# quzefan/LuSh-NeRF

Hardware: AMD Instinct MI355X
Metric: training rays/sec (fwd+bwd), N_samples=64+64 (higher is better)
Workload: dtype f16 MFMA forward (one fp16 plane per operand, fp32 accumulate; render outputs within 3e-5 of the fp32 reference); backward fp16 MFMA (one plane, per-launch power-of-two loss scale), fp32 accumulate; 1 GPU; poster_lushnerf 1xMI355X N_rand=4096/GPU N_samples=64 N_importance=64 blur kernel (DSK/RBK) on, fwd+bwd+Adam, one RCCL all-reduce of the flat gradient (BASELINE config C2); rays_per_gpu=4096, marched_rays_per_gpu=20480, planes_fwd=fp16x1, parallelism=dp1

## Files before the change

lush_nerf_amd/csrc/lush_mlp_wide.hip:

```cpp
#include "lush_mlp_wide.h"
#include "lush_host.h"

#include <cstdio>
#include <cstdlib>
#include <utility>

namespace lush {

constexpr int WD_PE_PITCH = PE_ROW * 2 + 16;
constexpr int WD_PE_PLANE = WD_MT * WD_PE_PITCH;
constexpr int WD_SB = 2;
enum { WB_NONE = 0, WB_REG = 1, WB_PEX = 2, WB_PED = 3 };
enum { WC_NONE = 0, WC_ACT = 1, WC_ALPHA = 2 };

constexpr int WD_WRAP = NetNerf::fwd4_len / 8;
static_assert(NetNerf::fwd4_len % 8 == 0, "the quarter-row stream is whole positions");

LUSH_CLOCK_DECL(lush_clock_wide_fwd)

struct WdRt {
    bool pre_on;
    unsigned clamp;
    char* mptr[2];
    unsigned lane2;
    const float* nextbias;
    char* tile;
    char* srows;
    unsigned soff[2];
    unsigned srow_off;
};

typedef __attribute__((ext_vector_type(2))) unsigned short u16x2;
struct WdConvTmp {
    unsigned o[4];
    unsigned m;
    unsigned word[4];
};

template <int NRQP, int KB0, bool MASK>
struct WdConv {
    static constexpr int NB = 2 * NRQP;
    static constexpr int UPT = MASK ? 8 : 4;
    static constexpr int UPB = 2 * UPT;
    static constexpr int NVU = NB * UPB;

    template <int K>
    static __device__ __forceinline__ void unit(f32x16 (&pend)[2][2], u32x4 (&xout)[2][16], WdConvTmp& t, unsigned clamp) {
        constexpr int b = K / UPB, r = K % UPB, tt = r / UPT, u = r % UPT;
        constexpr int c = b % 2, rbl = b / 2, kb = KB0 + 2 * rbl + tt;
        constexpr int kind = MASK ? ((u == 0 || u == 1 || u == 3 || u == 5) ? 0 : 1) : 0;
        constexpr int i = MASK ? (kind == 0 ? (u == 0 ? 0 : (u == 1 ? 1 : (u == 3 ? 2 : 3))) : (u == 2 ? 0 : (u == 4 ? 1 : (u == 6 ? 2 : 3)))) : u;
        if constexpr (kind == 0) {
            unsigned o;
            asm volatile("v_cvt_pk_f16_f32 %0, %1, %2\n\tv_pk_max_i16 %0, %0, %3"
                         : "=&v"(o) : "v"(pend[c][rbl][8 * tt + 2 * i]), "v"(pend[c][rbl][8 * tt + 2 * i + 1]), "s"(clamp));
            t.o[i] = o;
            if constexpr (i == 3) {
                const u32x4 v = {t.o[0], t.o[1], t.o[2], t.o[3]};
                xout[c][kb] = v;
            }
        } else {
            constexpr int sh = 8 * tt + 2 * i;
            unsigned z;
            if constexpr (tt == 0 && i == 0) {
                asm volatile("v_pk_sub_u16 %0, 1, %1 op_sel_hi:[0,1] clamp" : "=v"(t.m) : "v"(t.o[i]));
            } else if constexpr (tt == 1 && i == 3) {
                unsigned w;
                asm volatile("v_pk_sub_u16 %1, 1, %3 op_sel_hi:[0,1] clamp\n\tv_lshl_or_b32 %2, %1, %4, %2\n\tv_lshrrev_b32 %1, 15, %2\n\tv_or_b32 %1, %1, %2\n\tv_not_b32 %0, %1"
                             : "=v"(w), "=&v"(z), "+v"(t.m) : "v"(t.o[i]), "n"(sh));
                t.word[b] = w;
            } else {
                asm volatile("v_pk_sub_u16 %0, 1, %2 op_sel_hi:[0,1] clamp\n\tv_lshl_or_b32 %1, %0, %3, %1" : "=&v"(z), "+v"(t.m) : "v"(t.o[i]), "n"(sh));
            }
        }
    }
};


template <int NRQ, int NPOS, int BMAIN, int KB0, int PRE, int CK, int NRQP, int CKB0, bool MASK, int NRQN, int D, int PQ, bool STASH, int LD>
struct WdPass {
    static constexpr int KBPP = 8 / NRQ;
    static constexpr int NG = NPOS * 16;
    static constexpr int DG = D < NG ? D : NG;
    using CV = WdConv<NRQP, CKB0, MASK>;
    static constexpr int NBLK = CK == WC_ACT ? CV::NB : 0;
    static constexpr int IPB = CK == WC_ACT ? CV::UPB + 5 : 0;
    static constexpr int NIT = NBLK * IPB;
    static_assert(BMAIN == WB_REG || NPOS == 1, "a PE-image segment is one position");
    static_assert(!STASH || NPOS == 4, "the stash pipeline is laid out over the 16 positions of a layer");

    struct Regs {
        bf16x8 a1[4];
        u32x4 bpe[2][4];
        WdConvTmp ct;
        unsigned dma_dst, dma_off;
    };

    static constexpr int ST_JOBS = 8;
    static constexpr bool st_write(int g) { return STASH && g % 16 >= 12 && (4 * PQ + g / 16) < ST_JOBS; }
    static constexpr bool st_read(int g) { return STASH && g % 16 >= 12 && (4 * PQ + g / 16) >= 1 && (4 * PQ + g / 16) <= ST_JOBS; }
    static constexpr int st_store_job(int g) {
        const int P = 4 * PQ + g / 16, m = g % 16;
        const int J = m >= 14 ? P - 1 : (m < 2 ? P - 2 : -1);
        return (STASH && J >= 0 && J < ST_JOBS) ? J : -1;
    }
    static constexpr int st_store_row(int g) { return g % 16 >= 14 ? g % 16 - 14 : g % 16 + 2; }
    static constexpr bool st_store(int g) { return st_store_job(g) >= 0; }

    static constexpr int item_weight(int k) {
        const int r = k % (IPB > 0 ? IPB : 1), b = k / (IPB > 0 ? IPB : 1);
        if (r < CV::UPB) {
            if (!MASK) return 3;
            const int u = r % CV::UPT;
            return (u == 0 || u == 1 || u == 3 || u == 5) ? 3 : 2;
        }
        if (r == CV::UPB) return MASK ? 2 : 0;
        return (b / 2) < NRQN ? 1 : 0;
    }
    static constexpr int fixed_load(int g) {
        const int m = g % 16;
        int w = 0;
        if (m < 4) w += 1;
        if (m == 4 || m == 5) w += 3;
        if (m == 8) w += 10;
        if (m >= 9 && m <= 11) w += 1;
        if (st_write(g)) w += 1;
        if (st_read(g)) w += 1;
        if (st_store(g)) w += 2;
        return w;
    }
    struct Sched {
        int first[NG + 1];
        int cap;
    };
    static constexpr Sched make_sched() {
        Sched S{};
        for (int cap = 6; cap < 64; ++cap) {
            int k = 0;
            for (int g = 0; g < NG; ++g) {
                S.first[g] = k;
                int load = fixed_load(g);
                if (g < DG || g == NG - 1) {
                    while (k < NIT) {
                        const int w = item_weight(k);
                        if (w > 0 && load + w > cap && !(g == NG - 1)) break;
                        load += w;
                        ++k;
                    }
                }
            }
            S.first[NG] = k;
            S.cap = cap;
            int last = 0;
            for (int g = 0; g < NG; ++g)
                if (S.first[g + 1] > S.first[g]) last = g;
            if (k == NIT && (last < DG || NIT == 0)) return S;
        }
        return S;
    }
    static constexpr Sched SC = make_sched();

    template <int SRC, int NKB>
    static __device__ __forceinline__ void load_bpe(Regs& r, const char* peimg, int row0, int lane) {
        const int n = lane & 31, hh = lane >> 5;
        const char* p = peimg + (row0 + n) * WD_PE_PITCH + hh * 16;
#pragma unroll
        for (int c = 0; c < 2; ++c)
#pragma unroll
            for (int k = 0; k < NKB; ++k)
                r.bpe[c][k] = *reinterpret_cast<const u32x4*>(p + c * 32 * WD_PE_PITCH + ((SRC == WB_PED ? PE_X / 8 : 0) + 2 * k) * 16);
    }

    template <int SRC, int NRQ_, int I, int M>
    static __device__ __forceinline__ void mfma(f32x16 (&act)[2][2], const Regs& r, const WdCarry& cr, const u32x4 (&xin)[2][16]) {
        constexpr int u = M / 2, c = M % 2;
        constexpr int kbl = NRQ_ == 2 ? u / 2 : u, rbl = NRQ_ == 2 ? u % 2 : 0;
        const bf16x8 a = u < 4 ? cr.a0[u] : r.a1[u - 4];
        if constexpr (SRC == WB_REG) act[c][rbl] = mfma_f16(a, __builtin_bit_cast(bf16x8, xin[c][KB0 + I * (8 / NRQ_) + kbl]), act[c][rbl]);
        else act[c][rbl] = mfma_f16(a, __builtin_bit_cast(bf16x8, r.bpe[c][SRC == WB_PED ? kbl % 2 : kbl]), act[c][rbl]);
    }

    template <int M>
    static __device__ __forceinline__ void fixed(WdCtx& cx, Regs& r, WdCarry& cr, const char* rd, const char* rd_next) {
        if constexpr (M < 4) {
            r.a1[M] = *reinterpret_cast<const bf16x8*>(rd + (4 + M) * 1024 + cx.lane * 16);
        } else if constexpr (M == 4) {
            r.dma_dst = cx.dma_base + cx.slot_off;
            r.dma_off = cx.fetch_off;
        } else if constexpr (M == 5) {
            cx.fetch_off = cx.fetch_off + WD_SLOT == (unsigned)WD_WRAP * WD_SLOT ? 0u : cx.fetch_off + WD_SLOT;
            cx.slot_off = cx.slot_off + WD_SLOT == (unsigned)WD_S * WD_SLOT ? 0u : cx.slot_off + WD_SLOT;
        } else if constexpr (M == 8) {
            wd_dma_pair(cx.gbase + r.dma_off, cx.gbase + r.dma_off + 4096u, cx.voff, r.dma_dst, r.dma_dst + 4096u);
            cr.a0[0] = *reinterpret_cast<const bf16x8*>(rd_next + cx.lane * 16);
        } else if constexpr (M >= 9 && M <= 11) {
            cr.a0[M - 8] = *reinterpret_cast<const bf16x8*>(rd_next + (M - 8) * 1024 + cx.lane * 16);
        }
    }

    template <int K>
    static __device__ __forceinline__ void item(f32x16 (&pend)[2][2], u32x4 (&xout)[2][16], Regs& r, const WdRt& rt, int lane) {
        constexpr int b = K / IPB, rr = K % IPB, c = b % 2, rbl = b / 2;
        if constexpr (rr < CV::UPB) {
            CV::template unit<b * CV::UPB + rr>(pend, xout, r.ct, rt.clamp);
        } else if constexpr (rr == CV::UPB) {
            if constexpr (MASK) *reinterpret_cast<unsigned short*>(rt.mptr[c] + rbl * 128 + rt.lane2) = (unsigned short)r.ct.word[b];
        } else if constexpr (rbl < NRQN) {
            constexpr int j = rr - CV::UPB;
            const f32x4 v = *reinterpret_cast<const f32x4*>(rt.nextbias + rbl * 32 + 8 * (lane >> 5) + (j == 1 ? 0 : j == 2 ? 4 : j == 3 ? 16 : 20));
#pragma unroll
            for (int e = 0; e < 4; ++e) pend[c][rbl][4 * (j - 1) + e] = v[e];
        }
    }

    template <int G>
    static __device__ __forceinline__ void pending(f32x16 (&pend)[2][2], u32x4 (&xout)[2][16], Regs& r, const WdRt& rt, int lane, float (&alpha)[2]) {
        if constexpr (CK == WC_ACT) {
            wd_unroll<SC.first[G], SC.first[G + 1]>([&](auto kc) __attribute__((always_inline)) { item<decltype(kc)::value>(pend, xout, r, rt, lane); });
        } else if constexpr (CK == WC_ALPHA) {
            if constexpr (G == 0) {
                alpha[0] = pend[0][0][0];
                alpha[1] = pend[1][0][0];
            }
            if constexpr (G == 1) {
                asm volatile("" ::"v"(pend[0][0]), "v"(pend[1][0]));
            }
            if constexpr (G >= 1 && G <= 8) {
                constexpr int q = G - 1, c = q % 2, rbl = (q / 2) % 2, jj = q / 4;
                if constexpr (rbl < NRQN) {
#pragma unroll
                    for (int j2 = 0; j2 < 2; ++j2) {
                        const int j = 1 + 2 * jj + j2;
                        const f32x4 v = *reinterpret_cast<const f32x4*>(rt.nextbias + rbl * 32 + 8 * (lane >> 5) + (j == 1 ? 0 : j == 2 ? 4 : j == 3 ? 16 : 20));
#pragma unroll
                        for (int e = 0; e < 4; ++e) pend[c][rbl][4 * (j - 1) + e] = v[e];
                    }
                }
            }
        }
    }

    template <int JOB, int I4>
    static __device__ __forceinline__ void stash_store(const WdCarry& cr, const WdRt& rt) {
        constexpr int c = JOB / 4, j = JOB % 4;
        __builtin_nontemporal_store(cr.sb[I4 % WD_SB], reinterpret_cast<u32x4*>(rt.srows + ((c * 32 + 8 * I4) * LD + j * 64) * 2 + rt.srow_off));
    }
    template <int G>
    static __device__ __forceinline__ void stash(const u32x4 (&xin)[2][16], WdCarry& cr, const WdRt& rt, int lane) {
        constexpr int P = 4 * PQ + G / 16, m = G % 16;
        if constexpr (st_store(G)) stash_store<st_store_job(G), st_store_row(G)>(cr, rt);
        if constexpr (st_write(G)) {
            constexpr int job = P, c = job / 4, j = job % 4, o = m - 12;
            const int n = lane & 31, hh = lane >> 5;
            *reinterpret_cast<u32x4*>(rt.tile + (job % 2) * 4096 + n * 128 + (((2 * o + hh) ^ (n & 7)) << 4)) = xin[c][4 * j + o];
        }
        if constexpr (st_read(G)) {
            constexpr int job = P - 1, i = m - 12;
            const int row = 8 * i + (lane >> 3);
            cr.sb[i % WD_SB] = *reinterpret_cast<const u32x4*>(rt.tile + (job % 2) * 4096 + row * 128 + (((lane & 7) ^ (row & 7)) << 4));
        }
    }

    static constexpr int stores_in(int g0, int g1) {
        int n = 0;
        for (int g = g0 < 0 ? 0 : g0; g < g1 && g < NG; ++g) {
            if (st_store(g)) ++n;
            if (CK == WC_ACT && MASK)
                for (int k = SC.first[g]; k < SC.first[g + 1]; ++k)
                    if (k % IPB == CV::UPB) ++n;
        }
        return n;
    }

    template <int SRC, int NRQ_, int I, bool MAIN>
    static __device__ __forceinline__ void position(WdCtx& cx, f32x16 (&act)[2][2], f32x16 (&pend)[2][2], const u32x4 (&xin)[2][16],
                                                    u32x4 (&xout)[2][16], Regs& r, WdCarry& cr, const char* peimg, int row0, const WdRt& rt,
                                                    float (&alpha)[2]) {
        if constexpr (SRC != WB_REG) load_bpe<SRC, (SRC == WB_PED ? 2 : 4)>(r, peimg, row0, cx.lane);
        const char* rd = cx.ring + cx.slot_off;
        __builtin_amdgcn_sched_barrier(0);
        wd_unroll<0, 8>([&](auto mc) __attribute__((always_inline)) {
            constexpr int M = decltype(mc)::value;
            mfma<SRC, NRQ_, I, M>(act, r, cr, xin);
            fixed<M>(cx, r, cr, rd, nullptr);
            if constexpr (MAIN) {
                stash<16 * I + M>(xin, cr, rt, cx.lane);
                pending<16 * I + M>(pend, xout, r, rt, cx.lane, alpha);
            }
            __builtin_amdgcn_sched_barrier(0);
        });
        constexpr int younger = 2 * (WD_S - 2) + (MAIN ? stores_in(16 * (I + 1 - WD_S) + 8, 16 * I + 8) : 0);
        wd_wait_vm<(younger < 63 ? younger : 63)>();
        lds_barrier();
        const char* rd_next = cx.ring + cx.slot_off;
        __builtin_amdgcn_sched_barrier(0);
        wd_unroll<8, 16>([&](auto mc) __attribute__((always_inline)) {
            constexpr int M = decltype(mc)::value;
            mfma<SRC, NRQ_, I, M>(act, r, cr, xin);
            fixed<M>(cx, r, cr, rd, rd_next);
            if constexpr (MAIN) {
                stash<16 * I + M>(xin, cr, rt, cx.lane);
                pending<16 * I + M>(pend, xout, r, rt, cx.lane, alpha);
            }
            __builtin_amdgcn_sched_barrier(0);
        });
    }

    static __device__ __forceinline__ void run(WdCtx& cx, f32x16 (&act)[2][2], f32x16 (&pend)[2][2], const u32x4 (&xin)[2][16],
                                               u32x4 (&xout)[2][16], WdCarry& cr, const char* peimg, int row0, const WdRt& rt, float (&alpha)[2]) {
        Regs r;
        if constexpr (PRE == WB_PEX) {
            if (rt.pre_on) position<WB_PEX, 2, 0, false>(cx, act, pend, xin, xout, r, cr, peimg, row0, rt, alpha);
        } else if constexpr (PRE == WB_PED) {
            position<WB_PED, 2, 0, false>(cx, act, pend, xin, xout, r, cr, peimg, row0, rt, alpha);
        }
        wd_unroll<0, NPOS>([&](auto ic) __attribute__((always_inline)) {
            position<BMAIN, NRQ, decltype(ic)::value, true>(cx, act, pend, xin, xout, r, cr, peimg, row0, rt, alpha);
        });

    }
};

__device__ __noinline__ void wd_pe_tile(char* peimg, const float* rays, const float* z, int S, int P, long long tile_pt0, int tid, float* xd,
                                        const int* live) {
    const long long gpt = tile_pt0 + tid;
    float x[3] = {0.f, 0.f, 0.f}, d[3] = {0.f, 0.f, 0.f};
    if (gpt < P) point_of(rays, z, S, live ? (long long)live[gpt] : gpt, x, d);
    if (xd != nullptr) {
        float4* o = reinterpret_cast<float4*>(xd + gpt * 8);
        o[0] = make_float4(x[0], x[1], x[2], 0.f);
        o[1] = make_float4(d[0], d[1], d[2], 0.f);
    }
    float v[PE_X + PE_D];
#pragma unroll
    for (int c = 0; c < PE_X + PE_D; ++c) v[c] = 0.f;
#pragma unroll
    for (int i = 0; i < 3; ++i) {
        v[i] = x[i];
        v[PE_X + i] = d[i];
        float hx, lx, hd, ld;
        rev_split(x[i], &hx, &lx);
        rev_split(d[i], &hd, &ld);
#pragma unroll
        for (int k = 0; k < L_X; ++k) sincos_rev(hx, lx, k, &v[3 + 6 * k + i], &v[3 + 6 * k + 3 + i]);
#pragma unroll
        for (int k = 0; k < L_D; ++k) sincos_rev(hd, ld, k, &v[PE_X + 3 + 6 * k + i], &v[PE_X + 3 + 6 * k + 3 + i]);
    }
    char* row = peimg + tid * WD_PE_PITCH;
#pragma unroll
    for (int c = 0; c < (PE_X + PE_D) / 8; ++c) {
        u32x4 w;
#pragma unroll
        for (int j = 0; j < 4; ++j) {
            unsigned o[1];
            split_pair<1, DT_F16>(v[8 * c + 2 * j], v[8 * c + 2 * j + 1], o);
            w[j] = o[0];
        }
        *reinterpret_cast<u32x4*>(row + c * 16) = w;
    }
}

__device__ __forceinline__ void wd_bias(f32x16 (&acc)[2][2], const float* b, int h, int nrq) {
#pragma unroll
    for (int c = 0; c < 2; ++c)
#pragma unroll
        for (int rbl = 0; rbl < 2; ++rbl) {
            if (rbl < nrq) {
                const f32x4* p = reinterpret_cast<const f32x4*>(b + rbl * 32 + 8 * h);
                const f32x4 v0 = p[0], v1 = p[1], v2 = p[4], v3 = p[5];
#pragma unroll
                for (int e = 0; e < 4; ++e) {
                    acc[c][rbl][e] = v0[e];
                    acc[c][rbl][4 + e] = v1[e];
                    acc[c][rbl][8 + e] = v2[e];
                    acc[c][rbl][12 + e] = v3[e];
                }
            }
        }
}

template <class N, int SPK>
__global__ __launch_bounds__(WD_NT) void mlp_wide_fwd_kernel(const MlpFwdArgs A) {
    static_assert(N::HW == 256 && N::NL == 8 && N::HV == 128, "the wide kernel is built for the 8x256 net");
    constexpr int HW = N::HW, HV = N::HV, NL = N::NL, NRB = N::NRB;
    constexpr int NBIAS = N::f32_w_rgb;
    constexpr bool MASK = SPK > 0;
    constexpr int ML_BYTES = NRB * 128;
    constexpr int CB_BYTES = N::n_mask_layers * ML_BYTES;
    LUSH_CLOCK_STAMP(lush_clock_wide_fwd, 0);
    extern __shared__ __attribute__((aligned(16))) char smem[];
    float* biasl = reinterpret_cast<float*>(smem);
    char* ring = smem + NBIAS * 4;
    char* stage = ring + WD_S * WD_SLOT;
    char* peimg = stage + 8 * 4096;

    const int tid = threadIdx.x, lane = tid & 63;
    const int w = __builtin_amdgcn_readfirstlane(tid >> 6);
    const int n = lane & 31, h = lane >> 5;
    const char* wbase = reinterpret_cast<const char*>(A.wpk);
    {
        const float* f32 = reinterpret_cast<const float*>(wbase + (long long)N::total_entries * 1024);
        for (int i = tid; i < NBIAS; i += WD_NT) biasl[i] = f32[i];
    }
    WdCtx cx;
    cx.ring = ring;
    cx.ring_lds = (unsigned)(size_t)(__attribute__((address_space(3))) char*)ring;
    cx.gbase = wbase + (long long)N::fwd4_base * 1024;
    cx.slot_off = 0;
    cx.fetch_off = (unsigned)(WD_S % WD_WRAP) * WD_SLOT;
    cx.dma_base = __builtin_amdgcn_readfirstlane(cx.ring_lds + (unsigned)w * 1024u);
    cx.w = w;
    cx.lane = lane;
    cx.voff = (unsigned)lane * 16u + (unsigned)w * 1024u;
#pragma unroll
    for (int j = 0; j < WD_S; ++j)
        wd_dma_pair(cx.gbase + (unsigned)j * WD_SLOT, cx.gbase + (unsigned)j * WD_SLOT + 4096u, cx.voff, cx.dma_base + (unsigned)j * WD_SLOT, cx.dma_base + (unsigned)j * WD_SLOT + 4096u);

    const int row0 = w * 64;
    WdRt rt;
    rt.tile = stage + w * 8192;
    rt.pre_on = false;
    rt.srows = nullptr;
#pragma unroll
    for (int c = 0; c < 2; ++c) rt.soff[c] = (unsigned)(((c * 32 + n) * HW + h * 8) * 2);
    rt.srow_off = (unsigned)(((lane >> 3) * HW + (lane & 7) * 8) * 2);
    rt.lane2 = (unsigned)lane * 2u;
    float alpha[2] = {0.f, 0.f};
    int P = A.P, n_tiles = A.n_tiles;
    if (A.live_cnt != nullptr) {
        P = __builtin_amdgcn_readfirstlane(*A.live_cnt);
        n_tiles = (P + WD_MT - 1) / WD_MT;
    }

    for (int tile = blockIdx.x; tile < n_tiles; tile += gridDim.x) {
        const long long pt0 = (long long)tile * WD_MT;
        const long long wpt = pt0 + row0;
        wd_pe_tile(peimg, A.rays, A.z, A.S, P, pt0, tid, (SPK > 0 && !A.pe_rows) ? A.xd : nullptr, A.live_idx);
        if (tile == (int)blockIdx.x) wd_wait_vm<2 * (WD_S - 1)>();
        else wd_wait_vm<2 * (WD_S - 1) + (SPK > 0 ? 17 : 1)>();
        lds_barrier();
        if (SPK > 0 && A.pe_rows) {
            for (int i = tid; i < WD_MT * 12; i += WD_NT) {
                const int c = i % 12, pt = i / 12;
                const uint4 v = *reinterpret_cast<const uint4*>(peimg + pt * WD_PE_PITCH + c * 16);
                *reinterpret_cast<uint4*>(A.pe + (pt0 + pt) * PE_ROW + c * 8) = v;
            }
        }
        {
            unsigned long long gb = (unsigned long long)cx.gbase;
            asm volatile("" : "+s"(gb));
            cx.gbase = (const char*)gb;
        }
        char* mbase[2];
#pragma unroll
        for (int c = 0; c < 2; ++c) mbase[c] = reinterpret_cast<char*>(A.mask) + (wpt / 32 + c) * CB_BYTES;
        char* mdummy = reinterpret_cast<char*>(A.mask_dummy);
        auto mset = [&](int ml, int rb, bool dummy) __attribute__((always_inline)) {
#pragma unroll
            for (int c = 0; c < 2; ++c) rt.mptr[c] = dummy ? mdummy + c * 256 : mbase[c] + ml * ML_BYTES + rb * 128;
        };

        f32x16 accA[2][2], accB[2][2];
        u32x4 B0[2][16], B1[2][16];
        WdCarry a0;
#pragma unroll
        for (int i = 0; i < 4; ++i) a0.a0[i] = *reinterpret_cast<const bf16x8*>(cx.ring + cx.slot_off + i * 1024 + lane * 16);
        const float* btr = biasl + N::f32_b_trunk;
        wd_bias(accA, btr, h, 2);
        wd_bias(accB, btr + 64, h, 2);

        rt.clamp = 0u;
        WdPass<2, 1, WB_PEX, 0, WB_NONE, WC_NONE, 2, 0, MASK, 2, 16, 0, false, HW>::run(cx, accA, accB, B0, B0, a0, peimg, row0, rt, alpha);
        mset(0, 0, false); rt.nextbias = btr + 128;
        WdPass<2, 1, WB_PEX, 0, WB_NONE, WC_ACT, 2, 0, MASK, 2, 16, 0, false, HW>::run(cx, accB, accA, B0, B0, a0, peimg, row0, rt, alpha);
        mset(0, 2, false); rt.nextbias = btr + 192;
        WdPass<2, 1, WB_PEX, 0, WB_NONE, WC_ACT, 2, 4, MASK, 2, 16, 0, false, HW>::run(cx, accA, accB, B0, B0, a0, peimg, row0, rt, alpha);
        mset(0, 4, false); rt.nextbias = btr + HW;
        WdPass<2, 1, WB_PEX, 0, WB_NONE, WC_ACT, 2, 8, MASK, 2, 16, 0, false, HW>::run(cx, accB, accA, B0, B0, a0, peimg, row0, rt, alpha);

        auto layer = [&](int l, u32x4 (&xin)[2][16], u32x4 (&xout)[2][16]) __attribute__((always_inline)) {
            const bool feat = l == NL;
            const float* bl = btr + l * HW;
            rt.pre_on = l == N::SKIP;
            rt.srows = reinterpret_cast<char*>(A.h0 + (long long)(l - 1) * A.h_stride + wpt * HW);
            rt.clamp = 0u; mset(l - 1, 6, false); rt.nextbias = bl + 64;
            WdPass<2, 4, WB_REG, 0, WB_PEX, WC_ACT, 2, 12, MASK, 2, 48, 0, (SPK > 0), HW>::run(cx, accA, accB, xin, xin, a0, peimg, row0, rt, alpha);
            rt.clamp = feat ? 0x80008000u : 0u;
            mset(l, 0, feat); rt.nextbias = bl + 128;
            WdPass<2, 4, WB_REG, 0, WB_PEX, WC_ACT, 2, 0, MASK, 2, 60, 1, (SPK > 0), HW>::run(cx, accB, accA, xin, xout, a0, peimg, row0, rt, alpha);
            mset(l, 2, feat); rt.nextbias = bl + 192;
            WdPass<2, 4, WB_REG, 0, WB_PEX, WC_ACT, 2, 4, MASK, 2, 60, 2, (SPK > 0), HW>::run(cx, accA, accB, xin, xout, a0, peimg, row0, rt, alpha);
            mset(l, 4, feat); rt.nextbias = feat ? biasl + N::f32_b_alpha : bl + HW;
            WdPass<2, 4, WB_REG, 0, WB_PEX, WC_ACT, 2, 8, MASK, 2, 60, 3, (SPK > 0), HW>::run(cx, accB, accA, xin, xout, a0, peimg, row0, rt, alpha);
        };
#pragma unroll 1
        for (int l2 = 0; l2 < NL / 2; ++l2) {
            layer(1 + 2 * l2, B0, B1);
            layer(2 + 2 * l2, B1, B0);
        }
        rt.pre_on = false;
        rt.clamp = 0x80008000u; mset(0, 0, true); rt.nextbias = biasl + N::f32_b_views;
        WdPass<1, 2, WB_REG, 0, WB_NONE, WC_ACT, 2, 12, MASK, 2, 32, 0, false, HW>::run(cx, accA, accB, B1, B0, a0, peimg, row0, rt, alpha);
        rt.nextbias = biasl + N::f32_b_views + 64;
        WdPass<2, 4, WB_REG, 0, WB_PED, WC_ALPHA, 1, 0, MASK, 2, 60, 0, false, HW>::run(cx, accB, accA, B0, B0, a0, peimg, row0, rt, alpha);
        rt.clamp = 0u; mset(NL, 0, false); rt.nextbias = biasl + N::f32_b_rgb;
        WdPass<2, 4, WB_REG, 0, WB_PED, WC_ACT, 2, 0, MASK, 1, 60, 0, false, HW>::run(cx, accA, accB, B0, B1, a0, peimg, row0, rt, alpha);
        {
            WdConvTmp ct;
            using CV = WdConv<2, 4, MASK>;
            mset(NL, 2, false);
            wd_unroll<0, CV::NVU>([&](auto kc) __attribute__((always_inline)) { CV::template unit<decltype(kc)::value>(accA, B1, ct, 0u); });
            if constexpr (MASK) {
#pragma unroll
                for (int b = 0; b < 4; ++b) *reinterpret_cast<unsigned short*>(rt.mptr[b % 2] + (b / 2) * 128 + rt.lane2) = (unsigned short)ct.word[b];
            }
        }
        if constexpr (SPK > 0) {
            char* hvrows = reinterpret_cast<char*>(A.hv + wpt * HV);
#pragma unroll
            for (int c = 0; c < 2; ++c)
#pragma unroll
                for (int j = 0; j < N::KKV / 4; ++j) {
#pragma unroll
                    for (int kq = 0; kq < 4; ++kq)
                        *reinterpret_cast<u32x4*>(rt.tile + n * 128 + (((2 * kq + h) ^ (n & 7)) << 4)) = B1[c][4 * j + kq];
#pragma unroll
                    for (int i = 0; i < 4; ++i) {
                        const int row = 8 * i + (lane >> 3);
                        const u32x4 v = *reinterpret_cast<const u32x4*>(rt.tile + row * 128 + (((lane & 7) ^ (row & 7)) << 4));
                        __builtin_nontemporal_store(v, reinterpret_cast<u32x4*>(hvrows + ((c * 32 + 8 * i) * HV + j * 64) * 2 + (unsigned)(((lane >> 3) * HV + (lane & 7) * 8) * 2)));
                    }
                }
        }
        WdPass<1, 1, WB_REG, 0, WB_NONE, WC_NONE, 2, 0, MASK, 2, 16, 0, false, HW>::run(cx, accB, accA, B1, B1, a0, peimg, row0, rt, alpha);
        if (h == 0) {
#pragma unroll
            for (int c = 0; c < 2; ++c) {
                const long long gpt = wpt + c * 32 + n;
                if (gpt < P && A.live_idx == nullptr) {
                    float4 o;
                    o.x = accB[c][0][0];
                    o.y = accB[c][0][1];
                    o.z = accB[c][0][2];
                    o.w = alpha[c];
                    *reinterpret_cast<float4*>(A.raw + gpt * 4) = o;
                }
            }
        }
    }
    wd_wait_vm<0>();
    LUSH_CLOCK_STAMP(lush_clock_wide_fwd, 1);
}

LUSH_CLOCK_EXPORT(lush_debug_clock_fwd, lush_clock_wide_fwd)
static_assert((NetNerf::f32_w_rgb * 4) % 16 == 0, "the ring behind the bias block stays 16-byte aligned");
size_t mlp_wide_fwd_lds_bytes() { return (size_t)WD_S * WD_SLOT + (size_t)WD_PE_PLANE + (size_t)NetNerf::f32_w_rgb * 4 + 8 * 4096; }

template <int SPK>
static int launch_wide_sp(const MlpFwdArgs& a, hipStream_t s) {
    auto k = mlp_wide_fwd_kernel<NetNerf, SPK>;
    const size_t lds = mlp_wide_fwd_lds_bytes();
    static KernelOnce once;
    int dev = 0, n_cu = 0;
    if (int rc = current_device_cus(dev, n_cu)) return rc;
    if (int rc = kernel_lds_once(once, dev, reinterpret_cast<const void*>(k), lds)) return rc;
    const int tiles = (a.n_tiles * 128 + WD_MT - 1) / WD_MT;
    MlpFwdArgs b = a;
    b.n_tiles = tiles;
    const int grid = tiles < n_cu ? tiles : n_cu;
    hipLaunchKernelGGL(k, dim3(grid), dim3(WD_NT), lds, s, b);
    LUSH_HIP(hipGetLastError());
    return 0;
}

int launch_mlp_wide_fwd(const MlpFwdArgs& a, hipStream_t s) {
    const int sp = a.write_stash ? a.stash_planes : 0;
    if (sp == 0) return launch_wide_sp<0>(a, s);
    if (sp == 1) return launch_wide_sp<1>(a, s);
    return set_error("launch_mlp_wide_fwd: one stash plane at most");
}

}
```

Baseline: 350,800 rays/s.

## Prefetch next tile's ray/point inputs into LDS via async global_load_lds

Measured after the change: 351,800 rays/s, median of 6. No clear change (+0.3%).

```diff
diff --git a/lush_nerf_amd/csrc/lush_mlp_wide.hip b/lush_nerf_amd/csrc/lush_mlp_wide.hip
--- a/lush_nerf_amd/csrc/lush_mlp_wide.hip
+++ b/lush_nerf_amd/csrc/lush_mlp_wide.hip
@@ -321,13 +321,77 @@
     }
 };
 
-__device__ __noinline__ void wd_pe_tile(char* peimg, const float* rays, const float* z, int S, int P, long long tile_pt0, int tid, float* xd,
-                                        const int* live) {
-    const long long gpt = tile_pt0 + tid;
-    float x[3] = {0.f, 0.f, 0.f}, d[3] = {0.f, 0.f, 0.f};
-    if (gpt < P) point_of(rays, z, S, live ? (long long)live[gpt] : gpt, x, d);
+constexpr int WD_PT_SLOT = (PE_X + PE_D) * 2;
+static_assert(WD_PT_SLOT + 32 <= WD_PE_PITCH && WD_PT_SLOT % 16 == 0, "the point slot lies in the row's padding");
+constexpr int WD_PT_DWORDS = 11;
+static_assert(WD_PT_DWORDS * 256 <= 8192, "the fetch lands in the wave's own transposition tile");
+
+struct WdPoint { float z, o[3], dir[3], vd[3]; };
+
+__device__ __forceinline__ void wd_dma_dword(const void* gptr, unsigned lds_base) {
+    unsigned keep;
+    asm volatile("s_mov_b32 %0, m0\n\ts_mov_b32 m0, %2\n\ts_nop 0\n\tglobal_load_lds_dword %1, off\n\ts_mov_b32 m0, %0"
+                 : "=&s"(keep) : "v"(gptr), "s"(lds_base) : "memory");
+}
+__device__ __forceinline__ void wd_point_xd(const WdPoint& f, float (&x)[3], float (&d)[3]) {
+#pragma unroll
+    for (int i = 0; i < 3; ++i) {
+        x[i] = __fadd_rn(f.o[i], __fmul_rn(f.dir[i], f.z));
+        d[i] = f.vd[i];
+    }
+}
+
+__device__ __forceinline__ void wd_pe_tile(char* peimg, const float* rays, const float* z, int S, int P, int tile_pt0, int tile_step, bool first,
+                                           int tid, float* xd, const int* live, const char* land, unsigned land_lds) {
+    const int gpt = tile_pt0 + tid;
+    char* row = peimg + tid * WD_PE_PITCH;
+    const int nxt1 = gpt + tile_step < P ? gpt + tile_step : P - 1;
+    const int nxt2 = nxt1 + tile_step < P ? nxt1 + tile_step : P - 1;
+    float x[3], d[3];
+    int idx1;
+    WdPoint f;
+    if (first) {
+        int idx0 = gpt < P ? gpt : P - 1;
+        idx1 = nxt1;
+        if (live) {
+            idx0 = live[idx0];
+            idx1 = live[nxt1];
+        }
+        const float* rr = rays + (long long)(idx0 / S) * 11;
+        f.z = z[idx0];
+#pragma unroll
+        for (int i = 0; i < 3; ++i) {
+            f.o[i] = rr[i];
+            f.dir[i] = rr[3 + i];
+            f.vd[i] = rr[8 + i];
+        }
+        wd_point_xd(f, x, d);
+        asm volatile("" : "+v"(x[0]), "+v"(x[1]), "+v"(x[2]), "+v"(d[0]), "+v"(d[1]), "+v"(d[2]), "+v"(idx1));
+    } else {
+        const u32x4 s0 = *reinterpret_cast<const u32x4*>(row + WD_PT_SLOT), s1 = *reinterpret_cast<const u32x4*>(row + WD_PT_SLOT + 16);
+        const unsigned sx0 = s0[0], sx1 = s0[1], sx2 = s0[2], sd0 = s0[3], sd1 = s1[0], sd2 = s1[1], si = s1[2];
+        x[0] = __uint_as_float(sx0); x[1] = __uint_as_float(sx1); x[2] = __uint_as_float(sx2);
+        d[0] = __uint_as_float(sd0); d[1] = __uint_as_float(sd1); d[2] = __uint_as_float(sd2);
+        idx1 = (int)si;
+    }
+    {
+        const float* rr = rays + (long long)(idx1 / S) * 11;
+        wd_dma_dword(z + idx1, land_lds);
+#pragma unroll
+        for (int i = 0; i < 3; ++i) {
+            wd_dma_dword(rr + i, land_lds + (1 + i) * 256);
+            wd_dma_dword(rr + 3 + i, land_lds + (4 + i) * 256);
+            wd_dma_dword(rr + 8 + i, land_lds + (7 + i) * 256);
+        }
+        if (live) wd_dma_dword(live + nxt2, land_lds + 10 * 256);
+    }
+    __builtin_amdgcn_sched_barrier(0);
+    if (gpt >= P) {
+#pragma unroll
+        for (int i = 0; i < 3; ++i) x[i] = d[i] = 0.f;
+    }
     if (xd != nullptr) {
-        float4* o = reinterpret_cast<float4*>(xd + gpt * 8);
+        float4* o = reinterpret_cast<float4*>(xd + (long long)gpt * 8);
         o[0] = make_float4(x[0], x[1], x[2], 0.f);
         o[1] = make_float4(d[0], d[1], d[2], 0.f);
     }
@@ -346,7 +410,6 @@
 #pragma unroll
         for (int k = 0; k < L_D; ++k) sincos_rev(hd, ld, k, &v[PE_X + 3 + 6 * k + i], &v[PE_X + 3 + 6 * k + 3 + i]);
     }
-    char* row = peimg + tid * WD_PE_PITCH;
 #pragma unroll
     for (int c = 0; c < (PE_X + PE_D) / 8; ++c) {
         u32x4 w;
@@ -358,6 +421,22 @@
         }
         *reinterpret_cast<u32x4*>(row + c * 16) = w;
     }
+    __builtin_amdgcn_sched_barrier(0);
+    wd_wait_vm<0>();
+    const float* lf = reinterpret_cast<const float*>(land) + (tid & 63);
+    f.z = lf[0];
+#pragma unroll
+    for (int i = 0; i < 3; ++i) {
+        f.o[i] = lf[(1 + i) * 64];
+        f.dir[i] = lf[(4 + i) * 64];
+        f.vd[i] = lf[(7 + i) * 64];
+    }
+    const int idx2 = live ? reinterpret_cast<const int*>(lf)[10 * 64] : nxt2;
+    wd_point_xd(f, x, d);
+    const u32x4 n0 = {__float_as_uint(x[0]), __float_as_uint(x[1]), __float_as_uint(x[2]), __float_as_uint(d[0])};
+    const u32x4 n1 = {__float_as_uint(d[1]), __float_as_uint(d[2]), (unsigned)idx2, 0u};
+    *reinterpret_cast<u32x4*>(row + WD_PT_SLOT) = n0;
+    *reinterpret_cast<u32x4*>(row + WD_PT_SLOT + 16) = n1;
 }
 
 __device__ __forceinline__ void wd_bias(f32x16 (&acc)[2][2], const float* b, int h, int nrq) {
@@ -419,6 +498,7 @@
     const int row0 = w * 64;
     WdRt rt;
     rt.tile = stage + w * 8192;
+    const unsigned land_lds = __builtin_amdgcn_readfirstlane(cx.ring_lds + (unsigned)(WD_S * WD_SLOT) + (unsigned)w * 8192u);
     rt.pre_on = false;
     rt.srows = nullptr;
 #pragma unroll
@@ -435,7 +515,8 @@
     for (int tile = blockIdx.x; tile < n_tiles; tile += gridDim.x) {
         const long long pt0 = (long long)tile * WD_MT;
         const long long wpt = pt0 + row0;
-        wd_pe_tile(peimg, A.rays, A.z, A.S, P, pt0, tid, (SPK > 0 && !A.pe_rows) ? A.xd : nullptr, A.live_idx);
+        wd_pe_tile(peimg, A.rays, A.z, A.S, P, tile * WD_MT, (int)gridDim.x * WD_MT, tile == (int)blockIdx.x, tid,
+                   (SPK > 0 && !A.pe_rows) ? A.xd : nullptr, A.live_idx, rt.tile, land_lds);
         if (tile == (int)blockIdx.x) wd_wait_vm<2 * (WD_S - 1)>();
         else wd_wait_vm<2 * (WD_S - 1) + (SPK > 0 ? 17 : 1)>();
         lds_barrier();
```
